# microsoft/AI2BMD

Hardware: NVIDIA H100
Metric: MD steps/sec (higher is better)
Workload: dtype f32

## Files before the change

ai2bmd_b200/csrc/k_edge_tc.cuh:

```cuda
#pragma once
#include "k_edge.cuh"
#include "tc_common.cuh"

namespace vb {

constexpr int TC_TE = 128;
constexpr int TC_STAGES = 2;
constexpr int TC_MAX_STAGES = 3;
constexpr int TC_SLABS = D / tc::SLAB_K;
static_assert((TC_SLABS & (TC_SLABS - 1)) == 0, "tc_slab rotates the slab order with a mask: TC_SLABS must be a power of two");
constexpr int TC_MAXJOBS = 12;
constexpr int TC_LT = D + LDS_PAD;
typedef float TcRow[TC_LT];

struct TcJob {
    const float* img;
    int accumulate;
};

struct TcShared {
    alignas(1024) uint8_t ring[TC_STAGES][tc::STAGE_BYTES];
    alignas(16) float tile[TC_TE][TC_LT];
    alignas(16) float abuf[TC_TE][TC_LT];
    EdgeMeta<TC_TE> meta;
// ... 440 lines not shown
#pragma unroll
                        for (int u = 0; u < 2; u++) {
                            const int row = g0 + rb + u;
                            const float4 dd = sh.meta.d[row];
                            const float4 Pf = ld4(&sh.tile[row][col]) + bb;
                            const float4 fp = silu4(Pf);
                            const float4 a1 = tir[u][0] * dd.x + tir[u][1] * dd.y + tir[u][2] * dd.z;
                            const float4 a2 = ujr[u][0] * dd.x + ujr[u][1] * dd.y + ujr[u][2] * dd.z;
                            const float4 wdot = (tir[u][0] - a1 * dd.x) * (ujr[u][0] - a2 * dd.x) + (tir[u][1] - a1 * dd.y) * (ujr[u][1] - a2 * dd.y) +
                                                (tir[u][2] - a1 * dd.z) * (ujr[u][2] - a2 * dd.z);
                            if (rb + u < grpw && row < nvalid) {
                                st4(P1 + (size_t)(e0 + row) * 3 * D + 2 * D + col, Pf);
                                st4(Fout + (size_t)(e0 + row) * D + col, fin[u] + fp * wdot);
                            }
                        }
                    }
                    handoff_arrive(H_EU);
                }
                TC_TLG(7);
            }
            csync();
            TC_TL(18);
            const int cch = threadIdx.x & (D - 1), grp = threadIdx.x >> 7;
            float bnd[2][3] = {{0.f, 0.f, 0.f}, {0.f, 0.f, 0.f}};
            tc_fwd_s1(sh, ws, lw, VN, SP, sh.abuf, e0, nvalid, cch, grp, TC2_NGRP, bnd);
            TC_TL(19);
            tc_fwd_s2(sh, ws, lw, SP, sh.tile, e0, nvalid, cch, grp, TC2_NGRP, bnd);
            TC_TL(20);
        } else {
            const int cch = threadIdx.x & (D - 1), grp = threadIdx.x >> 7;
            const int rpw = (nvalid + TC2_CWARPS - 1) / TC2_CWARPS, r0 = warp * rpw;
            tc::mbar_wait(&sh.b_tile, tpar);
            csync();
            TC_TL(2);
            float Areg[RPW];
            tc2_mma(sh, ring, sh.abuf, acc, a.jobs[J_DK].accumulate, warp, lane, nvalid);
            TC_TL(4);
            tc2_acc_to(sh.tile, acc, warp, lane, nvalid);
            csync();
            {
                TC_TL(5);
                const float4 bb = ldg4(lw.b1 + col);
#pragma unroll
                for (int r = 0; r < RPW; r++) {
                    if (r >= rpw) break;
                    const int row = r0 + r;
                    const float4 qi = ldg4(QKV + (size_t)sh.meta.dst[row] * 3 * D + col);
                    const float4 kj = ldg4(QKV + (size_t)sh.meta.src[row] * 3 * D + D + col);
                    const float4 P = ld4(&sh.tile[row][col]) + bb;
                    const float av = quad_sum(hsum4(qi * kj * silu4(P)));
                    Areg[r] = silu_(av) * sh.meta.C[row];
                    if ((r < rpw && row < nvalid)) {
                        st4(P1 + (size_t)(e0 + row) * 3 * D + col, P);
                        if ((lane & 3) == 0) ATT[(size_t)(e0 + row) * H + (lane >> 2)] = av;
                    }
                }
            }
            TC_TL(6);
            tc2_mma(sh, ring, sh.abuf, acc, a.jobs[J_DV].accumulate, warp, lane, nvalid);
            TC_TL(7);
            csync();
            tc2_acc_to(sh.tile, acc, warp, lane, nvalid);
            csync();
            {
                TC_TL(8);
                const float4 bb = ldg4(lw.b1 + D + col);
#pragma unroll
                for (int r = 0; r < RPW; r++) {
                    if (r >= rpw) break;
                    const int row = r0 + r;
                    const float4 vj = ldg4(QKV + (size_t)sh.meta.src[row] * 3 * D + 2 * D + col);
                    const float4 P = ld4(&sh.tile[row][col]) + bb;
                    st4(&sh.tile[row][col], vj * silu4(P) * Areg[r]);
                    if ((r < rpw && row < nvalid)) st4(P1 + (size_t)(e0 + row) * 3 * D + D + col, P);
                }
            }
            csync();
            TC_TL(9);
            tc_fwd_xa(sh, ws, sh.tile, e0, nvalid, cch, grp, TC2_NGRP);
            TC_TL(10);
            if (upd) tc2_mma(sh, ring, sh.abuf, acc, a.jobs[J_F].accumulate, warp, lane, nvalid);
            tc2_tile_to_a(sh, nvalid);
            TC_TL(11);
            if (upd) {
                csync();
                tc2_acc_to(sh.tile, acc, warp, lane, nvalid);
                csync();
                const float4 bb = ldg4(lw.b1 + 2 * D + col);
#pragma unroll 1
                for (int rb = 0; rb < RPW; rb += 2) {
                    if (rb >= rpw) break;
                    float4 tir[2][3], ujr[2][3], fin[2];
#pragma unroll
                    for (int u = 0; u < 2; u++) {
                        const int row = r0 + rb + u;
                        const size_t i3 = (size_t)sh.meta.dst[row] * 3, j3 = (size_t)sh.meta.src[row] * 3;
                        if (rb + u < rpw && row < nvalid) fin[u] = ldg4(Fin + (size_t)(e0 + row) * D + col);
                        else fin[u] = f4s(0.f);
#pragma unroll
                        for (int s = 0; s < 3; s++) {
                            tir[u][s] = ldg4(TU + (i3 + s) * 2 * D + col);
                            ujr[u][s] = ldg4(TU + (j3 + s) * 2 * D + D + col);
                        }
                    }
#pragma unroll
                    for (int u = 0; u < 2; u++) {
                        const int row = r0 + rb + u;
                        const float4 dd = sh.meta.d[row];
                        const float4 Pf = ld4(&sh.tile[row][col]) + bb;
                        const float4 fp = silu4(Pf);
                        const float4 a1 = tir[u][0] * dd.x + tir[u][1] * dd.y + tir[u][2] * dd.z;
                        const float4 a2 = ujr[u][0] * dd.x + ujr[u][1] * dd.y + ujr[u][2] * dd.z;
                        const float4 wdot = (tir[u][0] - a1 * dd.x) * (ujr[u][0] - a2 * dd.x) + (tir[u][1] - a1 * dd.y) * (ujr[u][1] - a2 * dd.y) +
                                            (tir[u][2] - a1 * dd.z) * (ujr[u][2] - a2 * dd.z);
                        if ((rb + u < rpw && row < nvalid)) {
                            st4(P1 + (size_t)(e0 + row) * 3 * D + 2 * D + col, Pf);
                            st4(Fout + (size_t)(e0 + row) * D + col, fin[u] + fp * wdot);
                        }
                    }
                }
            }
            TC_TL(12);
            float bnd[2][3] = {{0.f, 0.f, 0.f}, {0.f, 0.f, 0.f}};
            tc2_mma(sh, ring, sh.abuf, acc, a.jobs[J_S1].accumulate, warp, lane, nvalid);
            TC_TL(13);
            csync();
            tc2_acc_to(sh.tile, acc, warp, lane, nvalid);
            csync();
            TC_TL(14);
            tc_fwd_s1(sh, ws, lw, VN, SP, sh.tile, e0, nvalid, cch, grp, TC2_NGRP, bnd);
            TC_TL(15);
            if (threadIdx.x == 0 && it + 1 < my_tiles) {
                const int en = ((int)blockIdx.x + (it + 1) * (int)gridDim.x) * trows;
                tc::tma_prefetch_l2(Fin + (size_t)en * D, (uint32_t)min(trows, E - en) * D * 4);
            }
            tc2_mma(sh, ring, sh.abuf, acc, a.jobs[J_S2].accumulate, warp, lane, nvalid);
            TC_TL(16);
            csync();
            tc2_acc_to(sh.tile, acc, warp, lane, nvalid);
            csync();
            TC_TL(17);
            tc_fwd_s2(sh, ws, lw, SP, sh.tile, e0, nvalid, cch, grp, TC2_NGRP, bnd);
            TC_TL(18);
        }
        csync();
    }
    if (a.tl != nullptr && blockIdx.x == 0 && threadIdx.x == 0) a.tl[31] = (unsigned long long)clock64();
}

}

namespace vb {

template <int ROWS>
__global__ void __launch_bounds__(TC2_THREADS, 1) edge_bwd_tc_kernel(const __grid_constant__ EdgeTcArgs a) {
    pdl_entry();
    extern __shared__ __align__(1024) uint8_t dyn_raw[];
    TcShared& sh = *tc_shared_base(dyn_raw);
    const Workspace& ws = a.ws;
    const int l = a.layer;
    const bool upd = (l < L - 1);
    const int J_G3A = 0, J_G3B = 1, J_G4DV = 2, J_G4DK = 3, J_G4F = 4;
    const int J_LAST = upd ? J_G4F : J_G4DK;
    constexpr int RPW = ROWS / TC2_CWARPS;
    constexpr int RB4 = (RPW % 4 == 0) ? 4 : 2;
    constexpr bool SMALL = ROWS <= 64;
    constexpr int RBM = SMALL ? 2 : RB4;
    const int warp = threadIdx.x >> 5, lane = threadIdx.x & 31, col = lane * 4, hd = lane >> 2;
    const int E = ws.rowptr[ws.N];
    const int trows = min(ROWS, max(16, a.tile_rows));
    const int ntiles_total = (E + trows - 1) / trows;
    const int my_tiles = ((int)blockIdx.x < ntiles_total) ? (ntiles_total - (int)blockIdx.x + (int)gridDim.x - 1) / (int)gridDim.x : 0;
    if (a.tl != nullptr && blockIdx.x == 0 && threadIdx.x == 0) a.tl[0] = (unsigned long long)clock64();
    TcRing<ROWS> ring;
    tc2_setup(sh, ring, a.jobs, a.njobs, my_tiles);
    if (a.tl != nullptr && blockIdx.x == 0 && threadIdx.x == 0) a.tl[1] = (unsigned long long)clock64();

    float acc[32];
    const float* __restrict__ QKV = ws.QKV[l];
    const float* __restrict__ VN = ws.VN[l];
    const float* __restrict__ TU = ws.TU[l];
    const float* __restrict__ P1 = ws.P1[l];
    const float* __restrict__ SP = ws.SP[l];
    const float* __restrict__ ATT = ws.ATT[l];
    const int cch = threadIdx.x & (D - 1), grp = threadIdx.x >> 7;
    for (int it = 0; it < my_tiles; it++) {
        const int e0 = ((int)blockIdx.x + it * (int)gridDim.x) * trows;
        const int nvalid = min(trows, E - e0);
        const int rpw = (nvalid + TC2_CWARPS - 1) / TC2_CWARPS, r0 = warp * rpw;
        load_edge_meta<TC_TE, TC2_CTHREADS>(sh.meta, ws, e0, nvalid);
        csync();
        TC_TL(2);
        if constexpr (SMALL) {
#pragma unroll 1
            for (int rb = 0; rb < RPW; rb += RB4) {
                if (rb >= rpw) break;
                float4 sp[RB4][2], gM[RB4][3], vn[RB4][3];
#pragma unroll
                for (int u = 0; u < RB4; u++) {
                    const int row = r0 + rb + u;
                    const size_t e = (size_t)(e0 + ((rb + u < rpw && row < nvalid) ? row : 0));
                    const size_t i3 = (size_t)sh.meta.dst[row] * 3, j3 = (size_t)sh.meta.src[row] * 3;
                    sp[u][0] = ldg4(SP + e * 2 * D + col);
                    sp[u][1] = ldg4(SP + e * 2 * D + D + col);
#pragma unroll
                    for (int s = 0; s < 3; s++) { gM[u][s] = ldg4(ws.GVEC + (i3 + s) * D + col); vn[u][s] = ldg4(VN + (j3 + s) * D + col); }
                }
#pragma unroll
                for (int u = 0; u < RB4; u++) {
                    const int row = r0 + rb + u;
                    const bool mine = rb + u < rpw, ok = (mine && row < nvalid);
                    const size_t j3 = (size_t)sh.meta.src[row] * 3;
                    const float4 dd = sh.meta.d[row];
                    const float4 s1 = silu4(sp[u][0]), s2 = silu4(sp[u][1]);
                    const float4 gs1 = gM[u][0] * vn[u][0] + gM[u][1] * vn[u][1] + gM[u][2] * vn[u][2];
                    const float gx_ = warp_sum(hsum4(gM[u][0] * s2)), gy_ = warp_sum(hsum4(gM[u][1] * s2)), gz_ = warp_sum(hsum4(gM[u][2] * s2));
                    if (mine) {
                        st4(&sh.abuf[row][col], ok ? gs1 * dsilu4(sp[u][0]) : f4s(0.f));
                        st4(&sh.tile[row][col], ok ? (gM[u][0] * dd.x + gM[u][1] * dd.y + gM[u][2] * dd.z) * dsilu4(sp[u][1]) : f4s(0.f));
                        if (lane == 0) { sh.eacc[row][1] = gx_; sh.eacc[row][2] = gy_; sh.eacc[row][3] = gz_; }
                    }
                    if (ok) {
                        red4(ws.GVNMSG + (j3 + 0) * D + col, gM[u][0] * s1);
                        red4(ws.GVNMSG + (j3 + 1) * D + col, gM[u][1] * s1);
                        red4(ws.GVNMSG + (j3 + 2) * D + col, gM[u][2] * s1);
                    }
                }
            }
            TC_TL(3);
        } else {
#pragma unroll 1
            for (int rb = 0; rb < RPW; rb += RB4) {
                if (rb >= rpw) break;
                float4 sp[RB4], gM[RB4][3], vn[RB4][3];
#pragma unroll
                for (int u = 0; u < RB4; u++) {
                    const int row = r0 + rb + u;
                    const size_t e = (size_t)(e0 + ((rb + u < rpw && row < nvalid) ? row : 0));
                    const size_t i3 = (size_t)sh.meta.dst[row] * 3, j3 = (size_t)sh.meta.src[row] * 3;
                    sp[u] = ldg4(SP + e * 2 * D + col);
#pragma unroll
                    for (int s = 0; s < 3; s++) { gM[u][s] = ldg4(ws.GVEC + (i3 + s) * D + col); vn[u][s] = ldg4(VN + (j3 + s) * D + col); }
                }
#pragma unroll
                for (int u = 0; u < RB4; u++) {
                    const int row = r0 + rb + u;
                    const bool ok = (rb + u < rpw && row < nvalid);
                    const size_t j3 = (size_t)sh.meta.src[row] * 3;
                    const float4 s1 = silu4(sp[u]);
                    const float4 gs1 = gM[u][0] * vn[u][0] + gM[u][1] * vn[u][1] + gM[u][2] * vn[u][2];
                    if (rb + u < rpw) st4(&sh.abuf[row][col], ok ? gs1 * dsilu4(sp[u]) : f4s(0.f));
                    if (ok) {
                        red4(ws.GVNMSG + (j3 + 0) * D + col, gM[u][0] * s1);
                        red4(ws.GVNMSG + (j3 + 1) * D + col, gM[u][1] * s1);
                        red4(ws.GVNMSG + (j3 + 2) * D + col, gM[u][2] * s1);
                    }
                }
            }
            TC_TL(3);
#pragma unroll 4
            for (int r = 0; r < RPW; r++) {
                if (r >= rpw) break;
                const int row = r0 + r;
                const bool ok = (r < rpw && row < nvalid);
                const size_t e = (size_t)(e0 + (ok ? row : 0));
                const size_t i3 = (size_t)sh.meta.dst[row] * 3;
                const float4 dd = sh.meta.d[row];
                const float4 sp = ldg4(SP + e * 2 * D + D + col);
                const float4 s2 = silu4(sp);
                const float4 gM0 = ldg4(ws.GVEC + (i3 + 0) * D + col), gM1 = ldg4(ws.GVEC + (i3 + 1) * D + col),
                             gM2 = ldg4(ws.GVEC + (i3 + 2) * D + col);
                const float gx_ = warp_sum(hsum4(gM0 * s2)), gy_ = warp_sum(hsum4(gM1 * s2)), gz_ = warp_sum(hsum4(gM2 * s2));
                if (lane == 0) { sh.eacc[row][1] = gx_; sh.eacc[row][2] = gy_; sh.eacc[row][3] = gz_; }
                st4(&sh.tile[row][col], ok ? (gM0 * dd.x + gM1 * dd.y + gM2 * dd.z) * dsilu4(sp) : f4s(0.f));
            }
            TC_TL(5);
        }
        csync();
        tc2_mma(sh, ring, sh.abuf, acc, a.jobs[J_G3A].accumulate, warp, lane, nvalid);
        TC_TL(6);
        if constexpr (!SMALL) {
            tc2_tile_to_a(sh, nvalid);
            TC_TL(7);
        }
        tc2_mma(sh, ring, SMALL ? sh.tile : sh.abuf, acc, a.jobs[J_G3B].accumulate, warp, lane, nvalid);
        TC_TL(8);
        csync();
        tc2_acc_to(sh.tile, acc, warp, lane, nvalid);
        csync();
        TC_TL(9);
#pragma unroll 1
        for (int rb = 0; rb < RPW; rb += RBM) {
            if (rb >= rpw) break;
            float4 gxa[RBM], vjr[RBM], pdvr[RBM];
            float avr[RBM];
#pragma unroll
            for (int u = 0; u < RBM; u++) {
                const int row = r0 + rb + u;
                const size_t e = (size_t)(e0 + ((rb + u < rpw && row < nvalid) ? row : 0));
                gxa[u] = load_gxa(ws, (size_t)sh.meta.dst[row], col);
                vjr[u] = ldg4(QKV + (size_t)sh.meta.src[row] * 3 * D + 2 * D + col);
                pdvr[u] = ldg4(P1 + e * 3 * D + D + col);
                avr[u] = (rb + u < rpw && row < nvalid) ? __ldg(ATT + e * H + hd) : 0.f;
            }
#pragma unroll
            for (int u = 0; u < RBM; u++) {
                const int row = r0 + rb + u;
                const bool ok = (rb + u < rpw && row < nvalid);
                const size_t j = sh.meta.src[row];
                const float Ce = sh.meta.C[row];
                const float av = avr[u], sa = silu_(av), A = sa * Ce;
                const bool mine = rb + u < rpw;
                const float4 gm = mine ? ld4(&sh.tile[row][col]) + gxa[u] : f4s(0.f);
                const float4 dv = silu4(pdvr[u]);
                if (mine) st4(&sh.abuf[row][col], ok ? gm * vjr[u] * A * dsilu4(pdvr[u]) : f4s(0.f));
                const float gA = quad_sum(hsum4(gm * vjr[u] * dv));
                if (mine && (lane & 3) == 0) sh.gattn[row][hd] = gA * Ce * dsilu_(av);
                const float gc = warp_sum((lane & 3) == 0 ? gA * sa : 0.f);
                if (mine && lane == 0) sh.eacc[row][0] = gc;
                if (ok) red4(ws.GQKV + j * 3 * D + 2 * D + col, gm * dv * A);
            }
        }
        TC_TL(10);
        csync();
#pragma unroll 1
        for (int rb = 0; rb < RPW; rb += RB4) {
            if (rb >= rpw) break;
            float4 pdkr[RB4], qir[RB4], kjr[RB4];
#pragma unroll
            for (int u = 0; u < RB4; u++) {
                const int row = r0 + rb + u;
                const size_t e = (size_t)(e0 + ((rb + u < rpw && row < nvalid) ? row : 0));
                pdkr[u] = ldg4(P1 + e * 3 * D + col);
                qir[u] = ldg4(QKV + (size_t)sh.meta.dst[row] * 3 * D + col);
                kjr[u] = ldg4(QKV + (size_t)sh.meta.src[row] * 3 * D + D + col);
            }
#pragma unroll
            for (int u = 0; u < RB4; u++) {
                const int row = r0 + rb + u;
                const bool ok = (rb + u < rpw && row < nvalid);
                const size_t j = sh.meta.src[row];
                const float4 dk = silu4(pdkr[u]);
                const float gav = sh.gattn[row][hd];
                if (rb + u < rpw) st4(&sh.tile[row][col], ok ? qir[u] * kjr[u] * gav * dsilu4(pdkr[u]) : f4s(0.f));
                if (SMALL && rb + u < rpw) st4(&tc_aux(sh)[row][col], kjr[u] * dk * gav);
                if (ok) red4(ws.GQKV + j * 3 * D + D + col, qir[u] * dk * gav);
            }
        }
        TC_TL(12);
        csync();
        tc2_mma(sh, ring, sh.abuf, acc, a.jobs[J_G4DV].accumulate, warp, lane, nvalid);
        TC_TL(13);
        if constexpr (!SMALL) {
            tc2_tile_to_a(sh, nvalid);
            TC_TL(14);
            csync();
#pragma unroll 4
            for (int r = 0; r < RPW; r++) {
                if (r >= rpw) break;
                const int row = r0 + r;
                const size_t e = (size_t)(e0 + ((r < rpw && row < nvalid) ? row : 0));
                const float4 dk = silu4(ldg4(P1 + e * 3 * D + col));
                const float4 kj = ldg4(QKV + (size_t)sh.meta.src[row] * 3 * D + D + col);
                st4(&sh.tile[row][col], kj * dk * sh.gattn[row][hd]);
            }
            csync();
        }
        {
            const TcRow* const gqb = SMALL ? tc_aux(sh) : sh.tile;
            const int i_first = sh.meta.dst[0], i_last = sh.meta.dst[nvalid - 1];
            for (int i = i_first + grp; i <= i_last; i += TC2_NGRP) {
                const int q0 = ws.rowptr[i], q1 = ws.rowptr[i + 1];
                const int lo = max(q0, e0) - e0, hi = min(q1, e0 + nvalid) - e0;
                float gq = 0.f;
                for (int r = lo; r < hi; r++) gq += gqb[r][cch];
                if (q0 >= e0 && q1 <= e0 + nvalid) ws.GQKV[(size_t)i * 3 * D + cch] = gq;
                else atomicAdd(ws.GQKV + (size_t)i * 3 * D + cch, gq);
            }
        }
        TC_TL(15);
        if (upd) {
            TcRow* const gpfb = SMALL ? sh.abuf : sh.tile;
            csync();
#pragma unroll 1
            for (int rb = 0; rb < RPW; rb += 2) {
                if (rb >= rpw) break;
                float4 gfr[2], pfr[2], tir[2][3], ujr[2][3];
#pragma unroll
                for (int u = 0; u < 2; u++) {
                    const int row = r0 + rb + u;
                    const bool ok = (rb + u < rpw && row < nvalid);
                    const size_t e = (size_t)(e0 + (ok ? row : 0));
                    const size_t i3 = (size_t)sh.meta.dst[row] * 3, j3 = (size_t)sh.meta.src[row] * 3;
                    gfr[u] = ok ? ld4(ws.GF + e * D + col) : f4s(0.f);
                    pfr[u] = ldg4(P1 + e * 3 * D + 2 * D + col);
#pragma unroll
                    for (int s = 0; s < 3; s++) {
                        tir[u][s] = ldg4(TU + (i3 + s) * 2 * D + col);
                        ujr[u][s] = ldg4(TU + (j3 + s) * 2 * D + D + col);
                    }
                }
#pragma unroll
                for (int u = 0; u < 2; u++) {
                    const int row = r0 + rb + u;
                    const bool ok = (rb + u < rpw && row < nvalid);
                    const size_t e = (size_t)(e0 + (ok ? row : 0));
                    const size_t j3 = (size_t)sh.meta.src[row] * 3;
                    const float4 dd = sh.meta.d[row];
                    const float4 gfn = gfr[u], pf = pfr[u];
                    const float4 fp = silu4(pf);
                    const float dv3[3] = {dd.x, dd.y, dd.z};
                    const float4 a1 = tir[u][0] * dd.x + tir[u][1] * dd.y + tir[u][2] * dd.z;
                    const float4 a2 = ujr[u][0] * dd.x + ujr[u][1] * dd.y + ujr[u][2] * dd.z;
                    float4 w1[3], w2[3];
#pragma unroll
                    for (int s = 0; s < 3; s++) { w1[s] = tir[u][s] - a1 * dv3[s]; w2[s] = ujr[u][s] - a2 * dv3[s]; }
                    const float4 wdot = w1[0] * w2[0] + w1[1] * w2[1] + w1[2] * w2[2];
                    const float4 gwd = gfn * fp;
                    if (rb + u < rpw) {
                        st4(&gpfb[row][col], gfn * wdot * dsilu4(pf));
                        if (SMALL) st4(&tc_aux(sh)[row][col], gwd);
                    }
                    const float4 c1 = gwd * (w2[0] * dd.x + w2[1] * dd.y + w2[2] * dd.z);
                    const float4 c2 = gwd * (w1[0] * dd.x + w1[1] * dd.y + w1[2] * dd.z);
                    float gdl[3];
                    float4 gu[3];
#pragma unroll
                    for (int s = 0; s < 3; s++) {
                        const float4 gw1 = gwd * w2[s], gw2 = gwd * w1[s];
                        gu[s] = gw2 - c2 * dv3[s];
                        gdl[s] = warp_sum(hsum4(tir[u][s] * c1 + a1 * gw1 + ujr[u][s] * c2 + a2 * gw2));
                    }
                    if (lane == 0 && rb + u < rpw) { sh.eacc[row][1] -= gdl[0]; sh.eacc[row][2] -= gdl[1]; sh.eacc[row][3] -= gdl[2]; }
                    if (ok) {
                        red4(ws.GTU + (j3 + 0) * 2 * D + D + col, gu[0]);
                        red4(ws.GTU + (j3 + 1) * 2 * D + D + col, gu[1]);
                        red4(ws.GTU + (j3 + 2) * 2 * D + D + col, gu[2]);
                    }
                    (void)e;
                }
            }
            TC_TL(16);
            csync();
            tc2_mma(sh, ring, SMALL ? sh.tile : sh.abuf, acc, a.jobs[J_G4DK].accumulate, warp, lane, nvalid);
            TC_TL(17);
            if constexpr (!SMALL) {
                tc2_tile_to_a(sh, nvalid);
                TC_TL(18);
                csync();
#pragma unroll 4
                for (int r = 0; r < RPW; r++) {
                    if (r >= rpw) break;
                    const int row = r0 + r;
                    const bool ok = (r < rpw && row < nvalid);
                    const size_t e = (size_t)(e0 + (ok ? row : 0));
                    const float4 gfn = ok ? ld4(ws.GF + e * D + col) : f4s(0.f);
                    st4(&sh.tile[row][col], gfn * silu4(ldg4(P1 + e * 3 * D + 2 * D + col)));
                }
                csync();
            }
            {
                const TcRow* const gwb = SMALL ? tc_aux(sh) : sh.tile;
                const int i_first = sh.meta.dst[0], i_last = sh.meta.dst[nvalid - 1];
                for (int i = i_first + grp; i <= i_last; i += TC2_NGRP) {
                    const int q0 = ws.rowptr[i], q1 = ws.rowptr[i + 1];
                    const int lo = max(q0, e0) - e0, hi = min(q1, e0 + nvalid) - e0;
                    float gt0 = 0.f, gt1 = 0.f, gt2 = 0.f;
                    auto term = [&](int r, float u0, float u1, float u2) {
                        const float4 dd = sh.meta.d[r];
                        const float gw = gwb[r][cch];
                        const float a2 = u0 * dd.x + u1 * dd.y + u2 * dd.z;
                        const float w20 = u0 - a2 * dd.x, w21 = u1 - a2 * dd.y, w22 = u2 - a2 * dd.z;
                        const float wd = w20 * dd.x + w21 * dd.y + w22 * dd.z;
                        gt0 += gw * (w20 - wd * dd.x);
                        gt1 += gw * (w21 - wd * dd.y);
                        gt2 += gw * (w22 - wd * dd.z);
                    };
                    int r = lo;
                    for (; r + 4 <= hi; r += 4) {
                        float u[4][3];
#pragma unroll
                        for (int q = 0; q < 4; q++) {
                            const size_t j3 = (size_t)sh.meta.src[r + q] * 3;
                            u[q][0] = __ldg(TU + (j3 + 0) * 2 * D + D + cch);
                            u[q][1] = __ldg(TU + (j3 + 1) * 2 * D + D + cch);
                            u[q][2] = __ldg(TU + (j3 + 2) * 2 * D + D + cch);
                        }
#pragma unroll
                        for (int q = 0; q < 4; q++) term(r + q, u[q][0], u[q][1], u[q][2]);
                    }
                    for (; r < hi; r++) {
                        const size_t j3 = (size_t)sh.meta.src[r] * 3;
                        term(r, __ldg(TU + (j3 + 0) * 2 * D + D + cch), __ldg(TU + (j3 + 1) * 2 * D + D + cch),
                             __ldg(TU + (j3 + 2) * 2 * D + D + cch));
                    }
                    if (q0 >= e0 && q1 <= e0 + nvalid) {
                        ws.GTU[((size_t)i * 3 + 0) * 2 * D + cch] = gt0;
                        ws.GTU[((size_t)i * 3 + 1) * 2 * D + cch] = gt1;
                        ws.GTU[((size_t)i * 3 + 2) * 2 * D + cch] = gt2;
                    } else {
                        atomicAdd(ws.GTU + ((size_t)i * 3 + 0) * 2 * D + cch, gt0);
                        atomicAdd(ws.GTU + ((size_t)i * 3 + 1) * 2 * D + cch, gt1);
                        atomicAdd(ws.GTU + ((size_t)i * 3 + 2) * 2 * D + cch, gt2);
                    }
                }
            }
        }
        TC_TL(19);
        if (threadIdx.x < 3 && it + 1 < my_tiles) {
            const int en = ((int)blockIdx.x + (it + 1) * (int)gridDim.x) * trows;
            const uint32_t nn = (uint32_t)min(trows, E - en);
            if (threadIdx.x == 0) tc::tma_prefetch_l2(SP + (size_t)en * 2 * D, nn * 2 * D * 4);
            else if (threadIdx.x == 1) tc::tma_prefetch_l2(P1 + (size_t)en * 3 * D, nn * 3 * D * 4);
            else tc::tma_prefetch_l2(ATT + (size_t)en * H, nn * H * 4);
        }
        tc2_mma(sh, ring, (SMALL && !upd) ? sh.tile : sh.abuf, acc, a.jobs[J_LAST].accumulate, warp, lane, nvalid);
        TC_TL(20);
        if (!SMALL || !upd) csync();
        tc2_acc_to(sh.tile, acc, warp, lane, nvalid);
        csync();
        TC_TL(21);
#pragma unroll 4
        for (int r = 0; r < RPW; r++) {
            if (r >= rpw) break;
            const int row = r0 + r;
            if ((r < rpw && row < nvalid)) {
                float* g = ws.GF + (size_t)(e0 + row) * D + col;
                float4 v = ld4(&sh.tile[row][col]);
                if (upd) v = v + ld4(g);
                st4(g, v);
            }
        }
        if (threadIdx.x < nvalid) {
            float* ea = ws.eacc + (size_t)(e0 + threadIdx.x) * 4;
            st4(ea, ld4(ea) + ld4(&sh.eacc[threadIdx.x][0]));
        }
        TC_TL(22);
        csync();
    }
    if (a.tl != nullptr && blockIdx.x == 0 && threadIdx.x == 0) a.tl[31] = (unsigned long long)clock64();
}

}
```

Measured before the change: 1154.

## Warp-specialize small-tile edge backward to overlap MMA with elementwise stages

For the small-tile backward edge kernel, the code splits warps into MMA warps and compute warps. Named handoff barriers let the tensor-core GEMMs for the dv/dk/filter gradients run while other warps compute gq sums and the filter-gradient elementwise pass. The final accumulator is written straight to global GF instead of being staged through shared memory. Elementwise phases are factored into helper functions, which also restructures the large-tile path. This adds synchronization complexity and the risk of races between the warp groups.

```diff
diff --git a/ai2bmd_b200/csrc/k_edge_tc.cuh b/ai2bmd_b200/csrc/k_edge_tc.cuh
--- a/ai2bmd_b200/csrc/k_edge_tc.cuh
+++ b/ai2bmd_b200/csrc/k_edge_tc.cuh
@@ -616,6 +616,218 @@
 
 namespace vb {
 
+
+template <int CAP, int RB>
+__device__ __forceinline__ void tc_bwd_gm(TcShared& sh, const Workspace& ws, const float* __restrict__ QKV, const float* __restrict__ P1,
+                                          const float* __restrict__ ATT, const TcRow* gmb, TcRow* pdvb, int e0, int nvalid, int r0,
+                                          int rpw, int lane, int wait_id) {
+    const int col = lane * 4, hd = lane >> 2;
+#pragma unroll 1
+    for (int rb = 0; rb < CAP; rb += RB) {
+        if (rb >= rpw) break;
+        float4 gxa[RB], vjr[RB], pdvr[RB];
+        float avr[RB];
+#pragma unroll
+        for (int u = 0; u < RB; u++) {
+            const int row = r0 + rb + u;
+            const size_t e = (size_t)(e0 + ((rb + u < rpw && row < nvalid) ? row : 0));
+            gxa[u] = load_gxa(ws, (size_t)sh.meta.dst[row], col);
+            vjr[u] = ldg4(QKV + (size_t)sh.meta.src[row] * 3 * D + 2 * D + col);
+            pdvr[u] = ldg4(P1 + e * 3 * D + D + col);
+            avr[u] = (rb + u < rpw && row < nvalid) ? __ldg(ATT + e * H + hd) : 0.f;
+        }
+        if (wait_id > 0 && rb == 0) handoff_wait(wait_id);
+#pragma unroll
+        for (int u = 0; u < RB; u++) {
+            const int row = r0 + rb + u;
+            const bool ok = (rb + u < rpw && row < nvalid);
+            const size_t j = sh.meta.src[row];
+            const float Ce = sh.meta.C[row];
+            const float av = avr[u], sa = silu_(av), A = sa * Ce;
+            const bool mine = rb + u < rpw;
+            const float4 gm = mine ? ld4(&gmb[row][col]) + gxa[u] : f4s(0.f);
+            const float4 dv = silu4(pdvr[u]);
+            if (mine) st4(&pdvb[row][col], ok ? gm * vjr[u] * A * dsilu4(pdvr[u]) : f4s(0.f));
+            const float gA = quad_sum(hsum4(gm * vjr[u] * dv));
+            if (mine && (lane & 3) == 0) sh.gattn[row][hd] = gA * Ce * dsilu_(av);
+            const float gc = warp_sum((lane & 3) == 0 ? gA * sa : 0.f);
+            if (mine && lane == 0) sh.eacc[row][0] = gc;
+            if (ok) red4(ws.GQKV + j * 3 * D + 2 * D + col, gm * dv * A);
+        }
+    }
+}
+
+template <int CAP, int RB>
+__device__ __forceinline__ void tc_bwd_pdk(TcShared& sh, const Workspace& ws, const float* __restrict__ QKV, const float* __restrict__ P1,
+                                           TcRow* pdkb, TcRow* gqb, int e0, int nvalid, int r0, int rpw, int lane) {
+    const int col = lane * 4, hd = lane >> 2;
+#pragma unroll 1
+    for (int rb = 0; rb < CAP; rb += RB) {
+        if (rb >= rpw) break;
+        float4 pdkr[RB], qir[RB], kjr[RB];
+#pragma unroll
+        for (int u = 0; u < RB; u++) {
+            const int row = r0 + rb + u;
+            const size_t e = (size_t)(e0 + ((rb + u < rpw && row < nvalid) ? row : 0));
+            pdkr[u] = ldg4(P1 + e * 3 * D + col);
+            qir[u] = ldg4(QKV + (size_t)sh.meta.dst[row] * 3 * D + col);
+            kjr[u] = ldg4(QKV + (size_t)sh.meta.src[row] * 3 * D + D + col);
+        }
+#pragma unroll
+        for (int u = 0; u < RB; u++) {
+            const int row = r0 + rb + u;
+            const bool mine = rb + u < rpw, ok = (mine && row < nvalid);
+            const size_t j = sh.meta.src[row];
+            const float4 dk = silu4(pdkr[u]);
+            const float gav = mine ? sh.gattn[row][hd] : 0.f;
+            if (mine) st4(&pdkb[row][col], ok ? qir[u] * kjr[u] * gav * dsilu4(pdkr[u]) : f4s(0.f));
+            if (gqb != nullptr && mine) st4(&gqb[row][col], kjr[u] * dk * gav);
+            if (ok) red4(ws.GQKV + j * 3 * D + D + col, qir[u] * dk * gav);
+        }
+    }
+}
+
+template <int CAP>
+__device__ __forceinline__ void tc_bwd_pf(TcShared& sh, const Workspace& ws, const float* __restrict__ P1, const float* __restrict__ TU,
+                                          TcRow* pfb, TcRow* gwb, int e0, int nvalid, int r0, int rpw, int lane, int wait_id) {
+    const int col = lane * 4;
+#pragma unroll 1
+    for (int rb = 0; rb < CAP; rb += 2) {
+        if (rb >= rpw) break;
+        float4 gfr[2], pfr[2], tir[2][3], ujr[2][3];
+#pragma unroll
+        for (int u = 0; u < 2; u++) {
+            const int row = r0 + rb + u;
+            const bool ok = (rb + u < rpw && row < nvalid);
+            const size_t e = (size_t)(e0 + (ok ? row : 0));
+            const size_t i3 = (size_t)sh.meta.dst[row] * 3, j3 = (size_t)sh.meta.src[row] * 3;
+            gfr[u] = ok ? ld4(ws.GF + e * D + col) : f4s(0.f);
+            pfr[u] = ldg4(P1 + e * 3 * D + 2 * D + col);
+#pragma unroll
+            for (int s = 0; s < 3; s++) {
+                tir[u][s] = ldg4(TU + (i3 + s) * 2 * D + col);
+                ujr[u][s] = ldg4(TU + (j3 + s) * 2 * D + D + col);
+            }
+        }
+        if (wait_id > 0 && rb == 0) handoff_wait(wait_id);
+#pragma unroll
+        for (int u = 0; u < 2; u++) {
+            const int row = r0 + rb + u;
+            const bool mine = rb + u < rpw, ok = (mine && row < nvalid);
+            const size_t j3 = (size_t)sh.meta.src[row] * 3;
+            const float4 dd = sh.meta.d[row];
+            const float4 gfn = gfr[u], pf = pfr[u];
+            const float4 fp = silu4(pf);
+            const float dv3[3] = {dd.x, dd.y, dd.z};
+            const float4 a1 = tir[u][0] * dd.x + tir[u][1] * dd.y + tir[u][2] * dd.z;
+            const float4 a2 = ujr[u][0] * dd.x + ujr[u][1] * dd.y + ujr[u][2] * dd.z;
+            float4 w1[3], w2[3];
+#pragma unroll
+            for (int s = 0; s < 3; s++) { w1[s] = tir[u][s] - a1 * dv3[s]; w2[s] = ujr[u][s] - a2 * dv3[s]; }
+            const float4 wdot = w1[0] * w2[0] + w1[1] * w2[1] + w1[2] * w2[2];
+            const float4 gwd = gfn * fp;
+            if (mine) {
+                st4(&pfb[row][col], gfn * wdot * dsilu4(pf));
+                if (gwb != nullptr) st4(&gwb[row][col], gwd);
+            }
+            const float4 c1 = gwd * (w2[0] * dd.x + w2[1] * dd.y + w2[2] * dd.z);
+            const float4 c2 = gwd * (w1[0] * dd.x + w1[1] * dd.y + w1[2] * dd.z);
+            float gdl[3];
+            float4 gu[3];
+#pragma unroll
+            for (int s = 0; s < 3; s++) {
+                const float4 gw1 = gwd * w2[s], gw2 = gwd * w1[s];
+                gu[s] = gw2 - c2 * dv3[s];
+                gdl[s] = warp_sum(hsum4(tir[u][s] * c1 + a1 * gw1 + ujr[u][s] * c2 + a2 * gw2));
+            }
+            if (lane == 0 && mine) { sh.eacc[row][1] -= gdl[0]; sh.eacc[row][2] -= gdl[1]; sh.eacc[row][3] -= gdl[2]; }
+            if (ok) {
+                red4(ws.GTU + (j3 + 0) * 2 * D + D + col, gu[0]);
+                red4(ws.GTU + (j3 + 1) * 2 * D + D + col, gu[1]);
+                red4(ws.GTU + (j3 + 2) * 2 * D + D + col, gu[2]);
+            }
+        }
+    }
+}
+
+__device__ __forceinline__ void tc_bwd_gq_sums(const TcShared& sh, const Workspace& ws, const TcRow* gqb, int e0, int nvalid, int c,
+                                               int grp, int ngrp) {
+    const int i_first = sh.meta.dst[0], i_last = sh.meta.dst[nvalid - 1];
+    for (int i = i_first + grp; i <= i_last; i += ngrp) {
+        const int q0 = ws.rowptr[i], q1 = ws.rowptr[i + 1];
+        const int lo = max(q0, e0) - e0, hi = min(q1, e0 + nvalid) - e0;
+        float gq = 0.f;
+        for (int r = lo; r < hi; r++) gq += gqb[r][c];
+        if (q0 >= e0 && q1 <= e0 + nvalid) ws.GQKV[(size_t)i * 3 * D + c] = gq;
+        else atomicAdd(ws.GQKV + (size_t)i * 3 * D + c, gq);
+    }
+}
+__device__ __forceinline__ void tc_bwd_gt_sums(const TcShared& sh, const Workspace& ws, const float* __restrict__ TU, const TcRow* gwb,
+                                               int e0, int nvalid, int c, int grp, int ngrp) {
+    const int i_first = sh.meta.dst[0], i_last = sh.meta.dst[nvalid - 1];
+    for (int i = i_first + grp; i <= i_last; i += ngrp) {
+        const int q0 = ws.rowptr[i], q1 = ws.rowptr[i + 1];
+        const int lo = max(q0, e0) - e0, hi = min(q1, e0 + nvalid) - e0;
+        float gt0 = 0.f, gt1 = 0.f, gt2 = 0.f;
+        auto term = [&](int r, float u0, float u1, float u2) {
+            const float4 dd = sh.meta.d[r];
+            const float gw = gwb[r][c];
+            const float a2 = u0 * dd.x + u1 * dd.y + u2 * dd.z;
+            const float w20 = u0 - a2 * dd.x, w21 = u1 - a2 * dd.y, w22 = u2 - a2 * dd.z;
+            const float wd = w20 * dd.x + w21 * dd.y + w22 * dd.z;
+            gt0 += gw * (w20 - wd * dd.x);
+            gt1 += gw * (w21 - wd * dd.y);
+            gt2 += gw * (w22 - wd * dd.z);
+        };
+        int r = lo;
+        for (; r + 4 <= hi; r += 4) {
+            float u[4][3];
+#pragma unroll
+            for (int q = 0; q < 4; q++) {
+                const size_t j3 = (size_t)sh.meta.src[r + q] * 3;
+                u[q][0] = __ldg(TU + (j3 + 0) * 2 * D + D + c);
+                u[q][1] = __ldg(TU + (j3 + 1) * 2 * D + D + c);
+                u[q][2] = __ldg(TU + (j3 + 2) * 2 * D + D + c);
+            }
+#pragma unroll
+            for (int q = 0; q < 4; q++) term(r + q, u[q][0], u[q][1], u[q][2]);
+        }
+        for (; r < hi; r++) {
+            const size_t j3 = (size_t)sh.meta.src[r] * 3;
+            term(r, __ldg(TU + (j3 + 0) * 2 * D + D + c), __ldg(TU + (j3 + 1) * 2 * D + D + c), __ldg(TU + (j3 + 2) * 2 * D + D + c));
+        }
+        if (q0 >= e0 && q1 <= e0 + nvalid) {
+            ws.GTU[((size_t)i * 3 + 0) * 2 * D + c] = gt0;
+            ws.GTU[((size_t)i * 3 + 1) * 2 * D + c] = gt1;
+            ws.GTU[((size_t)i * 3 + 2) * 2 * D + c] = gt2;
+        } else {
+            atomicAdd(ws.GTU + ((size_t)i * 3 + 0) * 2 * D + c, gt0);
+            atomicAdd(ws.GTU + ((size_t)i * 3 + 1) * 2 * D + c, gt1);
+            atomicAdd(ws.GTU + ((size_t)i * 3 + 2) * 2 * D + c, gt2);
+        }
+    }
+}
+
+__device__ __forceinline__ void tc2_acc_to_global(float* __restrict__ dst, const float (&acc)[32], int warp, int lane, int nvalid, bool add) {
+    const int q = warp >> 2, r = (q & 1) * 64 + (warp & 3) * 16 + (lane >> 2), c = (q >> 1) * 64 + 2 * (lane & 3);
+    float2 old[8][2];
+#pragma unroll
+    for (int i = 0; i < 8; i++)
+#pragma unroll
+        for (int h = 0; h < 2; h++)
+            old[i][h] = (add && r + 8 * h < nvalid) ? *reinterpret_cast<const float2*>(dst + (size_t)(r + 8 * h) * D + c + 8 * i)
+                                                    : make_float2(0.f, 0.f);
+#pragma unroll
+    for (int i = 0; i < 8; i++)
+#pragma unroll
+        for (int h = 0; h < 2; h++) {
+            const float x = acc[4 * i + 2 * h], y = acc[4 * i + 2 * h + 1];
+            if (r + 8 * h < nvalid)
+                *reinterpret_cast<float2*>(dst + (size_t)(r + 8 * h) * D + c + 8 * i) = add ? make_float2(x + old[i][h].x, y + old[i][h].y)
+                                                                                          : make_float2(x, y);
+        }
+}
+
 template <int ROWS>
 __global__ void __launch_bounds__(TC2_THREADS, 1) edge_bwd_tc_kernel(const __grid_constant__ EdgeTcArgs a) {
     pdl_entry();
@@ -629,8 +841,7 @@
     constexpr int RPW = ROWS / TC2_CWARPS;
     constexpr int RB4 = (RPW % 4 == 0) ? 4 : 2;
     constexpr bool SMALL = ROWS <= 64;
-    constexpr int RBM = SMALL ? 2 : RB4;
-    const int warp = threadIdx.x >> 5, lane = threadIdx.x & 31, col = lane * 4, hd = lane >> 2;
+    const int warp = threadIdx.x >> 5, lane = threadIdx.x & 31, col = lane * 4;
     const int E = ws.rowptr[ws.N];
     const int trows = min(ROWS, max(16, a.tile_rows));
     const int ntiles_total = (E + trows - 1) / trows;
@@ -652,6 +863,15 @@
         const int e0 = ((int)blockIdx.x + it * (int)gridDim.x) * trows;
         const int nvalid = min(trows, E - e0);
         const int rpw = (nvalid + TC2_CWARPS - 1) / TC2_CWARPS, r0 = warp * rpw;
+        auto prefetch_next = [&]() {
+            if (threadIdx.x < 3 && it + 1 < my_tiles) {
+                const int en = ((int)blockIdx.x + (it + 1) * (int)gridDim.x) * trows;
+                const uint32_t nn = (uint32_t)min(trows, E - en);
+                if (threadIdx.x == 0) tc::tma_prefetch_l2(SP + (size_t)en * 2 * D, nn * 2 * D * 4);
+                else if (threadIdx.x == 1) tc::tma_prefetch_l2(P1 + (size_t)en * 3 * D, nn * 3 * D * 4);
+                else tc::tma_prefetch_l2(ATT + (size_t)en * H, nn * H * 4);
+            }
+        };
         load_edge_meta<TC_TE, TC2_CTHREADS>(sh.meta, ws, e0, nvalid);
         csync();
         TC_TL(2);
@@ -692,6 +912,54 @@
                 }
             }
             TC_TL(3);
+            csync();
+            enum : int { H_GQ = 3, H_PF };
+            TcRow* const xb = tc_aux(sh);
+            if (tc2_is_mma_warp(warp)) {
+                tc2_mma<ROWS, true>(sh, ring, sh.abuf, acc, a.jobs[J_G3A].accumulate, warp, lane, nvalid);
+                TC_TL(6);
+                tc2_mma<ROWS, true>(sh, ring, sh.tile, acc, a.jobs[J_G3B].accumulate, warp, lane, nvalid);
+                tc2_acc_to(xb, acc, warp, lane, nvalid);
+                TC_TL(8);
+            }
+            tc_bwd_gm<RPW, 2>(sh, ws, QKV, P1, ATT, xb, xb, e0, nvalid, r0, rpw, lane, 1);
+            TC_TL(10);
+            __syncwarp();
+            tc_bwd_pdk<RPW, RB4>(sh, ws, QKV, P1, sh.abuf, sh.tile, e0, nvalid, r0, rpw, lane);
+            TC_TL(12);
+            csync();
+            if (tc2_is_mma_warp(warp)) {
+                tc2_mma<ROWS, true>(sh, ring, xb, acc, a.jobs[J_G4DV].accumulate, warp, lane, nvalid);
+                TC_TL(13);
+                tc_bwd_gq_sums(sh, ws, sh.tile, e0, nvalid, cch, grp, TC2_NGRP);
+                if (upd) handoff_arrive(H_GQ);
+                TC_TL(15);
+                prefetch_next();
+                tc2_mma<ROWS, true>(sh, ring, sh.abuf, acc, a.jobs[J_G4DK].accumulate, warp, lane, nvalid);
+                TC_TL(17);
+                if (upd) {
+                    handoff_wait(H_PF);
+                    TC_TL(16);
+                    tc2_mma<ROWS, true>(sh, ring, xb, acc, a.jobs[J_G4F].accumulate, warp, lane, nvalid);
+                    TC_TL(20);
+                }
+                tc2_acc_to_global(ws.GF + (size_t)e0 * D, acc, warp, lane, nvalid, upd);
+                TC_TL(21);
+            } else {
+                tc_bwd_gq_sums(sh, ws, sh.tile, e0, nvalid, cch, grp, TC2_NGRP);
+                TC_TLG(0);
+                if (upd) {
+                    constexpr int GRPW = ROWS / (TC2_CWARPS / 2);
+                    const int gw = (warp >> 3) * 4 + (warp & 3), grpw = (nvalid + 7) / 8;
+                    tc_bwd_pf<GRPW>(sh, ws, P1, TU, xb, sh.tile, e0, nvalid, gw * grpw, grpw, lane, H_GQ);
+                    handoff_arrive(H_PF);
+                    TC_TLG(1);
+                }
+            }
+            csync();
+            TC_TL(24);
+            if (upd) tc_bwd_gt_sums(sh, ws, TU, sh.tile, e0, nvalid, cch, grp, TC2_NGRP);
+            TC_TL(19);
         } else {
 #pragma unroll 1
             for (int rb = 0; rb < RPW; rb += RB4) {
@@ -739,83 +1007,25 @@
                 st4(&sh.tile[row][col], ok ? (gM0 * dd.x + gM1 * dd.y + gM2 * dd.z) * dsilu4(sp) : f4s(0.f));
             }
             TC_TL(5);
-        }
-        csync();
-        tc2_mma(sh, ring, sh.abuf, acc, a.jobs[J_G3A].accumulate, warp, lane, nvalid);
-        TC_TL(6);
-        if constexpr (!SMALL) {
+            csync();
+            tc2_mma(sh, ring, sh.abuf, acc, a.jobs[J_G3A].accumulate, warp, lane, nvalid);
+            TC_TL(6);
             tc2_tile_to_a(sh, nvalid);
             TC_TL(7);
-        }
-        tc2_mma(sh, ring, SMALL ? sh.tile : sh.abuf, acc, a.jobs[J_G3B].accumulate, warp, lane, nvalid);
-        TC_TL(8);
-        csync();
-        tc2_acc_to(sh.tile, acc, warp, lane, nvalid);
-        csync();
-        TC_TL(9);
-#pragma unroll 1
-        for (int rb = 0; rb < RPW; rb += RBM) {
-            if (rb >= rpw) break;
-            float4 gxa[RBM], vjr[RBM], pdvr[RBM];
-            float avr[RBM];
-#pragma unroll
-            for (int u = 0; u < RBM; u++) {
-                const int row = r0 + rb + u;
-                const size_t e = (size_t)(e0 + ((rb + u < rpw && row < nvalid) ? row : 0));
-                gxa[u] = load_gxa(ws, (size_t)sh.meta.dst[row], col);
-                vjr[u] = ldg4(QKV + (size_t)sh.meta.src[row] * 3 * D + 2 * D + col);
-                pdvr[u] = ldg4(P1 + e * 3 * D + D + col);
-                avr[u] = (rb + u < rpw && row < nvalid) ? __ldg(ATT + e * H + hd) : 0.f;
-            }
-#pragma unroll
-            for (int u = 0; u < RBM; u++) {
-                const int row = r0 + rb + u;
-                const bool ok = (rb + u < rpw && row < nvalid);
-                const size_t j = sh.meta.src[row];
-                const float Ce = sh.meta.C[row];
-                const float av = avr[u], sa = silu_(av), A = sa * Ce;
-                const bool mine = rb + u < rpw;
-                const float4 gm = mine ? ld4(&sh.tile[row][col]) + gxa[u] : f4s(0.f);
-                const float4 dv = silu4(pdvr[u]);
-                if (mine) st4(&sh.abuf[row][col], ok ? gm * vjr[u] * A * dsilu4(pdvr[u]) : f4s(0.f));
-                const float gA = quad_sum(hsum4(gm * vjr[u] * dv));
-                if (mine && (lane & 3) == 0) sh.gattn[row][hd] = gA * Ce * dsilu_(av);
-                const float gc = warp_sum((lane & 3) == 0 ? gA * sa : 0.f);
-                if (mine && lane == 0) sh.eacc[row][0] = gc;
-                if (ok) red4(ws.GQKV + j * 3 * D + 2 * D + col, gm * dv * A);
-            }
-        }
-        TC_TL(10);
-        csync();
-#pragma unroll 1
-        for (int rb = 0; rb < RPW; rb += RB4) {
-            if (rb >= rpw) break;
-            float4 pdkr[RB4], qir[RB4], kjr[RB4];
-#pragma unroll
-            for (int u = 0; u < RB4; u++) {
-                const int row = r0 + rb + u;
-                const size_t e = (size_t)(e0 + ((rb + u < rpw && row < nvalid) ? row : 0));
-                pdkr[u] = ldg4(P1 + e * 3 * D + col);
-                qir[u] = ldg4(QKV + (size_t)sh.meta.dst[row] * 3 * D + col);
-                kjr[u] = ldg4(QKV + (size_t)sh.meta.src[row] * 3 * D + D + col);
-            }
-#pragma unroll
-            for (int u = 0; u < RB4; u++) {
-                const int row = r0 + rb + u;
-                const bool ok = (rb + u < rpw && row < nvalid);
-                const size_t j = sh.meta.src[row];
-                const float4 dk = silu4(pdkr[u]);
-                const float gav = sh.gattn[row][hd];
-                if (rb + u < rpw) st4(&sh.tile[row][col], ok ? qir[u] * kjr[u] * gav * dsilu4(pdkr[u]) : f4s(0.f));
-                if (SMALL && rb + u < rpw) st4(&tc_aux(sh)[row][col], kjr[u] * dk * gav);
-                if (ok) red4(ws.GQKV + j * 3 * D + D + col, qir[u] * dk * gav);
-            }
-        }
-        TC_TL(12);
-        csync();
-        tc2_mma(sh, ring, sh.abuf, acc, a.jobs[J_G4DV].accumulate, warp, lane, nvalid);
-        TC_TL(13);
-        if constexpr (!SMALL) {
+            tc2_mma(sh, ring, sh.abuf, acc, a.jobs[J_G3B].accumulate, warp, lane, nvalid);
+            TC_TL(8);
+            csync();
+            tc2_acc_to(sh.tile, acc, warp, lane, nvalid);
+            csync();
+            TC_TL(9);
+            tc_bwd_gm<RPW, RB4>(sh, ws, QKV, P1, ATT, sh.tile, sh.abuf, e0, nvalid, r0, rpw, lane, 0);
+            TC_TL(10);
+            csync();
+            tc_bwd_pdk<RPW, RB4>(sh, ws, QKV, P1, sh.tile, nullptr, e0, nvalid, r0, rpw, lane);
+            TC_TL(12);
+            csync();
+            tc2_mma(sh, ring, sh.abuf, acc, a.jobs[J_G4DV].accumulate, warp, lane, nvalid);
+            TC_TL(13);
             tc2_tile_to_a(sh, nvalid);
             TC_TL(14);
             csync();
@@ -826,89 +1036,18 @@
                 const size_t e = (size_t)(e0 + ((r < rpw && row < nvalid) ? row : 0));
                 const float4 dk = silu4(ldg4(P1 + e * 3 * D + col));
                 const float4 kj = ldg4(QKV + (size_t)sh.meta.src[row] * 3 * D + D + col);
-                st4(&sh.tile[row][col], kj * dk * sh.gattn[row][hd]);
-            }
-            csync();
-        }
-        {
-            const TcRow* const gqb = SMALL ? tc_aux(sh) : sh.tile;
-            const int i_first = sh.meta.dst[0], i_last = sh.meta.dst[nvalid - 1];
-            for (int i = i_first + grp; i <= i_last; i += TC2_NGRP) {
-                const int q0 = ws.rowptr[i], q1 = ws.rowptr[i + 1];
-                const int lo = max(q0, e0) - e0, hi = min(q1, e0 + nvalid) - e0;
-                float gq = 0.f;
-                for (int r = lo; r < hi; r++) gq += gqb[r][cch];
-                if (q0 >= e0 && q1 <= e0 + nvalid) ws.GQKV[(size_t)i * 3 * D + cch] = gq;
-                else atomicAdd(ws.GQKV + (size_t)i * 3 * D + cch, gq);
-            }
-        }
-        TC_TL(15);
-        if (upd) {
-            TcRow* const gpfb = SMALL ? sh.abuf : sh.tile;
-            csync();
-#pragma unroll 1
-            for (int rb = 0; rb < RPW; rb += 2) {
-                if (rb >= rpw) break;
-                float4 gfr[2], pfr[2], tir[2][3], ujr[2][3];
-#pragma unroll
-                for (int u = 0; u < 2; u++) {
-                    const int row = r0 + rb + u;
-                    const bool ok = (rb + u < rpw && row < nvalid);
-                    const size_t e = (size_t)(e0 + (ok ? row : 0));
-                    const size_t i3 = (size_t)sh.meta.dst[row] * 3, j3 = (size_t)sh.meta.src[row] * 3;
-                    gfr[u] = ok ? ld4(ws.GF + e * D + col) : f4s(0.f);
-                    pfr[u] = ldg4(P1 + e * 3 * D + 2 * D + col);
-#pragma unroll
-                    for (int s = 0; s < 3; s++) {
-                        tir[u][s] = ldg4(TU + (i3 + s) * 2 * D + col);
-                        ujr[u][s] = ldg4(TU + (j3 + s) * 2 * D + D + col);
-                    }
-                }
-#pragma unroll
-                for (int u = 0; u < 2; u++) {
-                    const int row = r0 + rb + u;
-                    const bool ok = (rb + u < rpw && row < nvalid);
-                    const size_t e = (size_t)(e0 + (ok ? row : 0));
-                    const size_t j3 = (size_t)sh.meta.src[row] * 3;
-                    const float4 dd = sh.meta.d[row];
-                    const float4 gfn = gfr[u], pf = pfr[u];
-                    const float4 fp = silu4(pf);
-                    const float dv3[3] = {dd.x, dd.y, dd.z};
-                    const float4 a1 = tir[u][0] * dd.x + tir[u][1] * dd.y + tir[u][2] * dd.z;
-                    const float4 a2 = ujr[u][0] * dd.x + ujr[u][1] * dd.y + ujr[u][2] * dd.z;
-                    float4 w1[3], w2[3];
-#pragma unroll
-                    for (int s = 0; s < 3; s++) { w1[s] = tir[u][s] - a1 * dv3[s]; w2[s] = ujr[u][s] - a2 * dv3[s]; }
-                    const float4 wdot = w1[0] * w2[0] + w1[1] * w2[1] + w1[2] * w2[2];
-                    const float4 gwd = gfn * fp;
-                    if (rb + u < rpw) {
-                        st4(&gpfb[row][col], gfn * wdot * dsilu4(pf));
-                        if (SMALL) st4(&tc_aux(sh)[row][col], gwd);
-                    }
-                    const float4 c1 = gwd * (w2[0] * dd.x + w2[1] * dd.y + w2[2] * dd.z);
-                    const float4 c2 = gwd * (w1[0] * dd.x + w1[1] * dd.y + w1[2] * dd.z);
-                    float gdl[3];
-                    float4 gu[3];
-#pragma unroll
-                    for (int s = 0; s < 3; s++) {
-                        const float4 gw1 = gwd * w2[s], gw2 = gwd * w1[s];
-                        gu[s] = gw2 - c2 * dv3[s];
-                        gdl[s] = warp_sum(hsum4(tir[u][s] * c1 + a1 * gw1 + ujr[u][s] * c2 + a2 * gw2));
-                    }
-                    if (lane == 0 && rb + u < rpw) { sh.eacc[row][1] -= gdl[0]; sh.eacc[row][2] -= gdl[1]; sh.eacc[row][3] -= gdl[2]; }
-                    if (ok) {
-                        red4(ws.GTU + (j3 + 0) * 2 * D + D + col, gu[0]);
-                        red4(ws.GTU + (j3 + 1) * 2 * D + D + col, gu[1]);
-                        red4(ws.GTU + (j3 + 2) * 2 * D + D + col, gu[2]);
-                    }
-                    (void)e;
-                }
-            }
-            TC_TL(16);
-            csync();
-            tc2_mma(sh, ring, SMALL ? sh.tile : sh.abuf, acc, a.jobs[J_G4DK].accumulate, warp, lane, nvalid);
-            TC_TL(17);
-            if constexpr (!SMALL) {
+                st4(&sh.tile[row][col], kj * dk * sh.gattn[row][lane >> 2]);
+            }
+            csync();
+            tc_bwd_gq_sums(sh, ws, sh.tile, e0, nvalid, cch, grp, TC2_NGRP);
+            TC_TL(15);
+            if (upd) {
+                csync();
+                tc_bwd_pf<RPW>(sh, ws, P1, TU, sh.tile, nullptr, e0, nvalid, r0, rpw, lane, 0);
+                TC_TL(16);
+                csync();
+                tc2_mma(sh, ring, sh.abuf, acc, a.jobs[J_G4DK].accumulate, warp, lane, nvalid);
+                TC_TL(17);
                 tc2_tile_to_a(sh, nvalid);
                 TC_TL(18);
                 csync();
@@ -922,77 +1061,26 @@
                     st4(&sh.tile[row][col], gfn * silu4(ldg4(P1 + e * 3 * D + 2 * D + col)));
                 }
                 csync();
-            }
-            {
-                const TcRow* const gwb = SMALL ? tc_aux(sh) : sh.tile;
-                const int i_first = sh.meta.dst[0], i_last = sh.meta.dst[nvalid - 1];
-                for (int i = i_first + grp; i <= i_last; i += TC2_NGRP) {
-                    const int q0 = ws.rowptr[i], q1 = ws.rowptr[i + 1];
-                    const int lo = max(q0, e0) - e0, hi = min(q1, e0 + nvalid) - e0;
-                    float gt0 = 0.f, gt1 = 0.f, gt2 = 0.f;
-                    auto term = [&](int r, float u0, float u1, float u2) {
-                        const float4 dd = sh.meta.d[r];
-                        const float gw = gwb[r][cch];
-                        const float a2 = u0 * dd.x + u1 * dd.y + u2 * dd.z;
-                        const float w20 = u0 - a2 * dd.x, w21 = u1 - a2 * dd.y, w22 = u2 - a2 * dd.z;
-                        const float wd = w20 * dd.x + w21 * dd.y + w22 * dd.z;
-                        gt0 += gw * (w20 - wd * dd.x);
-                        gt1 += gw * (w21 - wd * dd.y);
-                        gt2 += gw * (w22 - wd * dd.z);
-                    };
-                    int r = lo;
-                    for (; r + 4 <= hi; r += 4) {
-                        float u[4][3];
-#pragma unroll
-                        for (int q = 0; q < 4; q++) {
-                            const size_t j3 = (size_t)sh.meta.src[r + q] * 3;
-                            u[q][0] = __ldg(TU + (j3 + 0) * 2 * D + D + cch);
-                            u[q][1] = __ldg(TU + (j3 + 1) * 2 * D + D + cch);
-                            u[q][2] = __ldg(TU + (j3 + 2) * 2 * D + D + cch);
-                        }
-#pragma unroll
-                        for (int q = 0; q < 4; q++) term(r + q, u[q][0], u[q][1], u[q][2]);
-                    }
-                    for (; r < hi; r++) {
-                        const size_t j3 = (size_t)sh.meta.src[r] * 3;
-                        term(r, __ldg(TU + (j3 + 0) * 2 * D + D + cch), __ldg(TU + (j3 + 1) * 2 * D + D + cch),
-                             __ldg(TU + (j3 + 2) * 2 * D + D + cch));
-                    }
-                    if (q0 >= e0 && q1 <= e0 + nvalid) {
-                        ws.GTU[((size_t)i * 3 + 0) * 2 * D + cch] = gt0;
-                        ws.GTU[((size_t)i * 3 + 1) * 2 * D + cch] = gt1;
-                        ws.GTU[((size_t)i * 3 + 2) * 2 * D + cch] = gt2;
-                    } else {
-                        atomicAdd(ws.GTU + ((size_t)i * 3 + 0) * 2 * D + cch, gt0);
-                        atomicAdd(ws.GTU + ((size_t)i * 3 + 1) * 2 * D + cch, gt1);
-                        atomicAdd(ws.GTU + ((size_t)i * 3 + 2) * 2 * D + cch, gt2);
-                    }
-                }
-            }
-        }
-        TC_TL(19);
-        if (threadIdx.x < 3 && it + 1 < my_tiles) {
-            const int en = ((int)blockIdx.x + (it + 1) * (int)gridDim.x) * trows;
-            const uint32_t nn = (uint32_t)min(trows, E - en);
-            if (threadIdx.x == 0) tc::tma_prefetch_l2(SP + (size_t)en * 2 * D, nn * 2 * D * 4);
-            else if (threadIdx.x == 1) tc::tma_prefetch_l2(P1 + (size_t)en * 3 * D, nn * 3 * D * 4);
-            else tc::tma_prefetch_l2(ATT + (size_t)en * H, nn * H * 4);
-        }
-        tc2_mma(sh, ring, (SMALL && !upd) ? sh.tile : sh.abuf, acc, a.jobs[J_LAST].accumulate, warp, lane, nvalid);
-        TC_TL(20);
-        if (!SMALL || !upd) csync();
-        tc2_acc_to(sh.tile, acc, warp, lane, nvalid);
-        csync();
-        TC_TL(21);
+                tc_bwd_gt_sums(sh, ws, TU, sh.tile, e0, nvalid, cch, grp, TC2_NGRP);
+            }
+            TC_TL(19);
+            prefetch_next();
+            tc2_mma(sh, ring, sh.abuf, acc, a.jobs[J_LAST].accumulate, warp, lane, nvalid);
+            TC_TL(20);
+            csync();
+            tc2_acc_to(sh.tile, acc, warp, lane, nvalid);
+            csync();
+            TC_TL(21);
 #pragma unroll 4
-        for (int r = 0; r < RPW; r++) {
-            if (r >= rpw) break;
-            const int row = r0 + r;
-            if ((r < rpw && row < nvalid)) {
-                float* g = ws.GF + (size_t)(e0 + row) * D + col;
-                float4 v = ld4(&sh.tile[row][col]);
-                if (upd) v = v + ld4(g);
-                st4(g, v);
+            for (int r = 0; r < RPW; r++) {
+                if (r >= rpw) break;
+                const int row = r0 + r;
+                if ((r < rpw && row < nvalid)) {
+                    float* g = ws.GF + (size_t)(e0 + row) * D + col;
+                    float4 v = ld4(&sh.tile[row][col]);
+                    if (upd) v = v + ld4(g);
+                    st4(g, v);
+                }
             }
         }
         if (threadIdx.x < nvalid) {
```

Result: faster. 1173, median of 6 (+1.6%).
